# hellozhuo/svnet

Hardware: AMD Instinct MI355X
Metric: point-clouds/sec fwd+bwd, sv_dgcnn_cls B=32 N=1024 k=20 (higher is better)
Workload: dtype f32 (ternary bit-planes in the binarized layers); 1 GPU; sv_dgcnn_cls --binary fwd+loss+bwd, B=32 per GPU, N=1024, k=20; global_batch=32, parallelism=dp1, collective=none (1 rank), rccl_world=1, launch=hipGraph replay, binlinear=i8_mfma (>= 1024 rows) + xnor (head)

## Files before the change

include/svnet_hip.h:

```cpp
#ifndef SVNET_HIP_H
#define SVNET_HIP_H

#include <stddef.h>
#include <stdint.h>

#ifdef __cplusplus
extern "C" {
#endif

#define SVNET_OK 0
#define SVNET_E_ARG (-1)
#define SVNET_E_UNSUPPORTED (-2)
#define SVNET_E_WORKSPACE (-3)
#define SVNET_E_LAUNCH (-4)

#define SVNET_RED_SLICES 16
#define SVNET_SLICED_LEN(L) ((SVNET_RED_SLICES + 1) * (L) + 2)
int svnet_slices_sum_f32(float* buf, int64_t L, void* stream);
int svnet_slices_sum_f64(double* buf, int64_t L, void* stream);

#define SVNET_ABI_VERSION 425
int svnet_version(void);
const char* svnet_last_error(void);

typedef struct svnet_gate_fwd_job {
    const float* gin; const double* gin_f64; float* gin_out; float in_scale; const float* W0; const float* W2;
    int64_t B, Cin, H, Ov; float* h; float* gate;
    const float* rows; int64_t R;
} svnet_gate_fwd_job;
typedef struct svnet_gate_bwd_job {
    const float* dgate; const float* gate; const float* h; const float* gin; float in_scale; const float* W0; const float* W2;
    int64_t B, Cin, H, Ov; float out_scale; float* dgin; float* dW0; float* dW2;
} svnet_gate_bwd_job;

size_t svnet_knn_workspace_bytes(int64_t B, int64_t N, int64_t C);
int svnet_knn_f32(const float* x, int64_t B, int64_t N, int64_t C, int64_t sb, int64_t sn, int64_t sc,
                  int xx_mode, int k, int64_t* idx_out, void* workspace, size_t workspace_bytes, void* stream);
int svnet_knn_sv_f32(const float* s, int64_t Cs, const float* v, int64_t Cv3, int64_t B, int64_t N, int k, int64_t* idx_out,
                     void* workspace, size_t workspace_bytes, void* stream);

int svnet_knn_table_fusable(int64_t B, int64_t N, int64_t C);
int svnet_knn_from_table_f32(const void* workspace, size_t workspace_bytes, int64_t B, int64_t N, int64_t C, int k, int64_t* idx_out,
                             void* stream);
int svnet_edgeblock_apply_knn_f32(const int32_t* n_max, const int32_t* n_min, const float* mv, const float* mvn, const float* coef,
                                  const float* gate, int64_t P, int64_t N, int64_t Os, int64_t Ov, float slope, float* s_out, float* v_out,
                                  float* s_cat, int64_t s_ld, float* v_cat, int64_t v_ld, void* knn_workspace, size_t knn_workspace_bytes,
                                  void* stream);
int svnet_xyzblock_apply_knn_f32(const float* y_max, const float* y_min, const float* mv, const float* mvn, const float* coef,
                                 const float* gate, int64_t P, int64_t N, int64_t Os, int64_t Ov, float slope, float* s_out, float* v_out,
                                 float* s_cat, int64_t s_ld, float* v_cat, int64_t v_ld, void* knn_workspace, size_t knn_workspace_bytes,
                                 void* stream);

int svnet_edge_xyz_f32(const float* x, const int64_t* idx, int64_t B, int64_t N, int64_t k, int64_t m, int mode,
                       float* out, void* stream);

int svnet_edge_diffcat_fwd_f32(const float* table, const int64_t* idx, int idx_is_global, int64_t B, int64_t N,
                               int64_t k, int64_t G, int64_t F, float* out, void* stream);
int svnet_edge_diffcat_bwd_f32(const float* d_out, const int64_t* idx, int idx_is_global, int64_t B, int64_t N,
                               int64_t k, int64_t G, int64_t F, float* d_table, void* stream);

typedef struct svnet_gemm_desc {
    int64_t M, N, K;
    const float* A; int64_t a_rs, a_cs;
    const float* a_scale;
    const uint64_t* a_sign; const uint64_t* a_nz;
    const float* B; int64_t b_rs, b_cs;
    int b_exact;
    float* C; int64_t ldc, c_cs;
    float alpha;
    const float* col_scale;
    const float* bias;
    const uint64_t* mask;
    float* col_sum;
    int split_k;
// ... 391 lines not shown
```

svnet_amd/_ops.py:

```python
import ctypes

import torch

from . import _lib, config
from ._lib import BinHeadDesc, GemmDesc, call

BN_EPS = 1e-5
RED_SLICES = _lib.DEFINES["SVNET_RED_SLICES"]
BN_MOMENTUM = 0.1

TAP = None



def _p(t):
    return None if t is None else ctypes.c_void_p(t.data_ptr())


def _stream():
    return ctypes.c_void_p(torch.cuda.current_stream().cuda_stream)


def _hip(*tensors):
    for t in tensors:
# ... 1679 lines not shown
              and all(torch.is_tensor(b[0]) and torch.is_tensor(b[1]) and a[0] == b[0].data_ptr() and a[1] == b[1].data_ptr()
                      for a, b in zip(self.filled, levels)))
        if not ok:
            return torch.cat([x[0] for x in levels], dim=-1), torch.cat([x[1] for x in levels], dim=-1)
        flat = [t for vw in self.views for t in vw]
        return _CatFilled.apply(self.s, self.v, len(levels), *flat)


_SINK = None


class _CatFilled(torch.autograd.Function):

    @staticmethod
    def forward(ctx, s_cat, v_cat, n, *flat):
        ctx.ws = [flat[2 * i].shape[-1] for i in range(n)]
        ctx.wv = [flat[2 * i + 1].shape[-1] for i in range(n)]
        return s_cat.view(s_cat.shape), v_cat.view(v_cat.shape)

    @staticmethod
    def backward(ctx, gs, gv):
        out, so, vo = [], 0, 0
        for ws, wv in zip(ctx.ws, ctx.wv):
            out.append(gs[..., so:so + ws] if gs is not None else None)
            out.append(gv[..., vo:vo + wv] if gv is not None else None)
            so, vo = so + ws, vo + wv
        return (None, None, None) + tuple(out)


class EdgeBlock(torch.autograd.Function):

    @staticmethod
    def forward(ctx, s, v, idx, k, training, Wz, scz, W1, beta1, scale1, g1, b1, rm1, rv1, W2, sc2, g2, b2, rm2, rv2, Wg0, Wg2,
                nbt1=None, nbt2=None):
        _hip(s, v)
        from ._lib import EdgeBlockDesc
        s = _f32c(s)
        v = _f32c(v)
        B, N, Cs = s.shape
        Cv = v.shape[-1]
        Os, Ov = W1.shape[0], W2.shape[0]
        P, E = B * N, B * N * k
        dev = s.device
        f32 = dict(dtype=torch.float32, device=dev)
        W1c, W2c, Wzc, Wg0c, Wg2c = _f32c(W1), _f32c(W2), _f32c(Wz), _f32c(Wg0), _f32c(Wg2)
        sc1, sc2f, sczf = _f32c(scale1).reshape(-1), _f32c(sc2).reshape(-1), _f32c(scz).reshape(-1)

        import weakref
        refs = tuple(weakref.ref(p_) for p_ in (W1, beta1, W2, sc2, Wz, scz))

        def build():
            out = {"wv": torch.empty((2 * Ov + 6, Cv), **f32), "scv": torch.empty((2 * Ov + 6,), **f32),
                   "w_sign": torch.empty((Os, 5), dtype=torch.int64, device=dev), "w_nz": torch.empty((Os, 5), dtype=torch.int64, device=dev),
                   "beta_perm": torch.empty((5 * 64,), **f32), "wbt": torch.empty((320 * ((Os + 15) // 16 * 16),), dtype=torch.int16, device=dev),
                   "w_dense": torch.zeros((1,), dtype=torch.int32, device=dev)}

            def rebuild():
                ps = [r() for r in refs]
                if any(p_ is None for p_ in ps):
                    return
                W1p, beta1p, W2p, sc2p, Wzp, sczp = ps
                call("svnet_edgeblock_prepare_vec_f32", _p(_f32c(W2p.detach())), _p(_f32c(sc2p.detach()).reshape(-1)), _p(_f32c(Wzp.detach())),
                     _p(_f32c(sczp.detach()).reshape(-1)), Ov, Cv, _p(out["wv"]), _p(out["scv"]), _stream())
                call("svnet_edgeblock_prepare_f32", _p(_f32c(W1p.detach())), _p(_f32c(beta1p.detach())), Os, Cs, Cv, _p(out["w_sign"]), _p(out["w_nz"]),
                     _p(out["beta_perm"]), _stream())
                call("svnet_edgeblock_wbt_bf16", _p(out["w_sign"]), _p(out["w_nz"]), Os, Cs, Cv, _p(out["wbt"]), _p(out["w_dense"]), _stream())
            rebuild()
            return out, rebuild
        packed = PLANES.get("edge", (W1, beta1, W2, sc2, Wz, scz), build)
        wv, scv, w_sign, w_nz, beta_perm, wbt = (packed[n] for n in ("wv", "scv", "w_sign", "w_nz", "beta_perm", "wbt"))
        zz = torch.empty((P * 3, 6), **f32)
        ut = torch.empty((P * 3, 2 * Ov), **f32)
        main, side = torch.cuda.current_stream(dev), _side_stream(dev)
        side.wait_stream(main)
        idx = (idx if torch.is_tensor(idx) else idx.idx).contiguous()
        _hip(idx)
        with torch.cuda.stream(side):
            gemm(3 * P, 6, Cv, A=v, a_rs=Cv, a_cs=1, B=wv[2 * Ov:], b_rs=1, b_cs=Cv, b_exact=True, C=zz, ldc=6, col_scale=scv[2 * Ov:])
            gemm(3 * P, 2 * Ov, Cv, A=v, a_rs=Cv, a_cs=1, B=wv, b_rs=1, b_cs=Cv, b_exact=True, C=ut, ldc=2 * Ov, col_scale=scv)
        main.wait_stream(side)

        n_max = torch.empty((P, Os), dtype=torch.int32, device=dev)
        n_min = torch.empty((P, Os), dtype=torch.int32, device=dev)
        slot_max = torch.empty((P, Os), dtype=torch.uint8, device=dev)
        slot_min = torch.empty((P, Os), dtype=torch.uint8, device=dev)
        mv = torch.empty((P, 3, Ov), **f32)
        mvn = torch.empty((P, 3, Ov), **f32)
        if training:
            stat_n, stat_v, gate_sum = _zeros_pool(dev, ((RED_SLICES * 2 * Os,), torch.int64), ((RED_SLICES * 2 * Ov,), torch.float64),
                                                     ((B, 2 * Cs), torch.float64))
        else:
            stat_n = stat_v = None
            gate_sum = _zeros((B, 2 * Cs), torch.float64, dev)
        d = EdgeBlockDesc()
        d.B, d.N, d.k = B, N, k
        d.Cs, d.Cv, d.Os, d.Ov = Cs, Cv, Os, Ov
        d.s, d.v, d.idx, d.zz, d.ut = _p(s), _p(v), _p(idx), _p(zz), _p(ut)
        d.w_sign, d.w_nz, d.beta_perm = _p(w_sign), _p(w_nz), _p(beta_perm)
        d.w_dense = _p(packed["w_dense"]) if config.EDGE_DENSE_WEIGHTS else None
        d.n_max, d.n_min, d.slot_max, d.slot_min = _p(n_max), _p(n_min), _p(slot_max), _p(slot_min)
        d.mv, d.mvn, d.stat_n, d.stat_v, d.gate_sum = _p(mv), _p(mvn), _p(stat_n), _p(stat_v), _p(gate_sum)
        keep = (training and any(ctx.needs_input_grad)) or TAP is not None
        n16 = torch.empty((E, Os), dtype=torch.int16, device=dev) if keep else None
        planes = torch.empty((E, 15), dtype=torch.int64, device=dev) if keep else None
        d.n16, d.planes = _p(n16), _p(planes)
        call("svnet_edgeblock_fwd_f32", ctypes.byref(d), _stream())
        if TAP is not None:
# ... 263 lines not shown
```

svnet_amd/csrc/edgeblock_bwd.hip:

```cpp
#include <stdlib.h>

#include "bf16_split.h"
#include "common.h"
#include "gate_mlp.h"
#include "prelude.h"

namespace {

#define ATOMIC_ADD(p, v) do { if (MODE != 1) atomicAdd((p), (v)); else asm volatile("" :: "v"(v)); } while (0)

#ifdef SVNET_PHASE_CLOCK
#define PHASE_MARK(i) do { if (threadIdx.x == 0) { const long long t_ = clock64(); ph_acc[i] += (unsigned long long)(t_ - ph_t); ph_t = t_; } } while (0)
#define PHASE_INIT() __shared__ unsigned long long ph_acc[16]; long long ph_t = 0, ph_t0 = 0, ph_w0 = 0; \
    if (threadIdx.x == 0) { for (int i_ = 0; i_ < 16; ++i_) ph_acc[i_] = 0ull; ph_t = ph_t0 = clock64(); ph_w0 = wall_clock64(); }
#define PHASE_FLUSH() do { if (threadIdx.x == 0 && d.debug) { ph_acc[14] = (unsigned long long)(clock64() - ph_t0); \
        ph_acc[15] = (unsigned long long)(wall_clock64() - ph_w0); for (int i_ = 0; i_ < 16; ++i_) if (ph_acc[i_]) \
        atomicAdd(reinterpret_cast<unsigned long long*>(d.debug) + 8 + 16 * (blockIdx.x & 255) + i_, ph_acc[i_]); } } while (0)
#else
#define PHASE_MARK(i) do { } while (0)
#define PHASE_INIT() do { } while (0)
#define PHASE_FLUSH() do { } while (0)
#endif

typedef __attribute__((ext_vector_type(16))) float f32x16;

#ifndef SVNET_DN_PIECES
#define SVNET_DN_PIECES 3
#endif

constexpr float VEPS = 1e-6f;
constexpr int NW = 5;
constexpr int NCOL = NW * 64;
constexpr int TE = 32;
__host__ __device__ __forceinline__ int dx_stride(int Cs, int Cv) { return (2 * Cs + 6 * Cv) | 1; }

__host__ __device__ __forceinline__ int dn_stride(int Os) { return Os + 8; }

__device__ __forceinline__ int nth_set_bit10(uint32_t mask, int n) {
    int res = -1;
#pragma unroll
    for (int b = 9; b >= 0; --b) {
        const int below = __popc(mask & ((1u << b) - 1u));
        if (((mask >> b) & 1u) && below == n) res = b;
    }
    return res;
}
__global__ void edgeblock_wbt_kernel(const uint64_t* __restrict__ w_sign, const uint64_t* __restrict__ w_nz, int Os, int Cs, int Cv,
                                     uint16_t* __restrict__ wbt, uint32_t* __restrict__ w_dense) {
    if (w_dense && blockIdx.x == 0 && threadIdx.x < 64) {
        bool ok = true;
        for (int i = threadIdx.x; i < Os * NW; i += 64) {
            const int w = i % NW, nb = w < 2 ? Cs : 2 * Cv;
            const uint64_t used = nb >= 64 ? ~0ull : ((1ull << nb) - 1ull);
            ok = ok && ((w_nz[i] & used) == used);
        }
        const uint64_t bad = __ballot(!ok);
        if (threadIdx.x == 0) *w_dense = bad == 0ull ? 1u : 0u;
    }
    const int nks = (Os + 15) >> 4;
    const int total = (NCOL / 32) * nks * 512;
    for (int e = blockIdx.x * blockDim.x + threadIdx.x; e < total; e += gridDim.x * blockDim.x) {
        const int j = e & 7, ln = (e >> 3) & 63, rest = e >> 9;
        const int ct = rest / nks, ks = rest - ct * nks;
        const int col = ct * 32 + (ln & 31), o = ks * 16 + 8 * (ln >> 5) + j;
        const int w = col >> 6, b = col & 63;
        uint16_t val = 0;
        if (o < Os) {
            const uint64_t nz = w_nz[o * NW + w], sg = w_sign[o * NW + w];
            val = ((nz >> b) & 1ull) ? (((sg >> b) & 1ull) ? 0x3F80 : 0xBF80) : 0;
        }
        wbt[e] = val;
    }
}

__global__ __launch_bounds__(256) void edgeblock_bwd_prelude_kernel(
    const float* __restrict__ gs, const float* __restrict__ gv, const int32_t* __restrict__ n_max, const int32_t* __restrict__ n_min,
    const float* __restrict__ mv, const float* __restrict__ mvn, const float* __restrict__ coef, const float* __restrict__ scale1,
    const float* __restrict__ gate, int64_t P, int64_t N, int Os, int Ov, float slope, int64_t rows_per_block,
    float* __restrict__ gy, float* __restrict__ red, float* __restrict__ redv, float* __restrict__ dgate,
    const float* __restrict__ gs2, int64_t gs2_ld, const float* __restrict__ gv2, int64_t gv2_ld, float* __restrict__ gv_sum) {
    svnet_prelude_body<int32_t>(gs, gv, n_max, n_min, mv, mvn, coef, scale1, gate, P, N, Os, Ov, slope, rows_per_block, gy, red, redv, dgate, gs2,
                                gs2_ld, gv2, gv2_ld, gv_sum);
}

__global__ void edgeblock_bwd_coeffs_kernel(const float* __restrict__ red, const float* __restrict__ redv, const float* __restrict__ coef,
                                            const float* __restrict__ g1, const float* __restrict__ g2, int64_t E, int Os, int Ov,
                                            int training, const float* __restrict__ scale1, float* __restrict__ bcoef,
                                            float* __restrict__ dg1, float* __restrict__ db1, float* __restrict__ dg2,
                                            float* __restrict__ db2, svnet_gate_bwd_job job, int coef_blocks, int gate_chunks) {
    if ((int)blockIdx.x >= coef_blocks) {
        const int g = (int)blockIdx.x - coef_blocks;
        svnet_gate_bwd_block(job, g / gate_chunks, g % gate_chunks, gate_chunks);
        return;
    }
    const int c = blockIdx.x * blockDim.x + threadIdx.x;
    const float invE = 1.f / (float)E;
    if (c < Os) {
        const float iy = coef[3 * Os + c];
        float r0 = 0.f, r1 = 0.f;
#pragma unroll
        for (int sl = 0; sl < SVNET_RED_SLICES; ++sl) { r0 += red[sl * 2 * Os + c]; r1 += red[sl * 2 * Os + Os + c]; }
        const float m1 = training ? r0 * invE : 0.f, m2 = training ? r1 * invE : 0.f, cs = g1[c] * iy;
        bcoef[c] = m1;
        bcoef[Os + c] = m2;
        bcoef[2 * Os + c] = cs;
        dg1[c] = r1;
        db1[c] = r0;
        if (scale1) {
            float* chc = bcoef + ((3 * Os + 2 * Ov + 3) & ~3);
            const float sc = scale1[c], my = coef[2 * Os + c];
            chc[c] = cs;
            chc[Os + c] = cs * (m1 - my * iy * m2);
            chc[2 * Os + c] = cs * sc * iy * m2;
            chc[3 * Os + c] = sc;
            chc[4 * Os + c] = coef[c] >= 0.f ? 1.f : 0.f;
        }
    }
    if (c < Ov) {
        const float* Avp = coef + 4 * Os;
        const float mean = Avp[2 * Ov + c], is = Avp[3 * Ov + c];
// ... 174 lines not shown
    in.gp = in_range ? c.gp : 0u;
    if (in_range && c.gp != loaded_p) { load_point(d, c.gp, v2_lane, cm, pend); loaded_p = c.gp; }
    in.gj = in.valid ? c.b * N + (uint32_t)jloc : 0u;
    const uint32_t ld = (uint32_t)min(lane, (int)Cv - 1);
    const float* vj = d.v + in.gj * 3u * Cv;
    in.vj0 = ld_f32_sbase(vj, 4u * ld);
    in.vj1 = ld_f32_sbase(vj, 4u * (ld + Cv));
    in.vj2 = ld_f32_sbase(vj, 4u * (ld + 2u * Cv));
    const float* zj = d.zz + in.gj * 18u;
    in.zj[0] = zj[0];  in.zj[1] = zj[1];  in.zj[2] = zj[2];
    in.zj[3] = zj[6];  in.zj[4] = zj[7];  in.zj[5] = zj[8];
    in.zj[6] = zj[12]; in.zj[7] = zj[13]; in.zj[8] = zj[14];
}

#define SVNET_PHASEC_REQUESTS()                                                                             \
    do {                                                                                                    \
            const uint32_t Nu_ = (uint32_t)d.N, uCv_ = (uint32_t)Cv; \
            const int row0_ = 8 * wave, n3_ = 3 * Cv; \
            { \
                EdgeCursor c2; \
                cursor_init(d, tp, e0, row0_, c2); \
_Pragma("unroll") \
                for (int rr = 0; rr < 8; ++rr) { \
                    const int jl = __builtin_amdgcn_readlane(jv8, rr); \
                    const bool ok = c2.e < E && (uint32_t)jl < Nu_; \
                    const uint32_t gj = ok ? c2.b * Nu_ + (uint32_t)jl : 0u; \
                    const float* vr = d.v + gj * 3u * uCv_; \
                    pc_vst[rr][0] = ld_f32_sbase(vr, 4u * (uint32_t)min(lane, n3_ - 1)); \
                    if (NC2 > 44) pc_vst[rr][1] = ld_f32_sbase(vr, 4u * (uint32_t)min(lane + 64, n3_ - 1)); \
                    cursor_next(d, c2); \
                } \
            } \
            const int el_ = lane >> 3, ch_ = (lane >> 2) & 1, qq_ = min(lane & 3, 2); \
            const int rw_ = row0_ + el_; \
            const bool in_range_ = e0 + rw_ < E; \
            const uint32_t dq_ = small_div((uint32_t)(tp.t0 + rw_), tp.kmagic); \
            int pin_ = tp.pin0 + (int)dq_; \
            uint32_t b_ = tp.b0; \
            while (pin_ >= (int)Nu_) { pin_ -= (int)Nu_; ++b_; } \
            const int jloc_ = __builtin_amdgcn_ds_bpermute(4 * el_, jv8); \
            const bool valid_ = in_range_ && (uint32_t)jloc_ < Nu_; \
            const uint32_t gj_ = valid_ ? b_ * Nu_ + (uint32_t)jloc_ : 0u; \
            const uint32_t gpc_ = in_range_ ? tp.gp0 + dq_ : 0u; \
            const float* vip_ = d.v + (gpc_ * 3u + (uint32_t)qq_) * uCv_; \
_Pragma("unroll") \
            for (int i = 0; i < PC_NCH; ++i) pc_vi[i] = vip_[min(ch_ * PC_NCH + i, Cv - 1)]; \
            const float* zjp_ = d.zz + gj_ * 18u + (uint32_t)qq_ * 6u; \
            const float* zip_ = d.zz + gpc_ * 18u + (uint32_t)qq_ * 6u; \
            pc_zj[0] = zjp_[0]; pc_zj[1] = zjp_[1]; pc_zj[2] = zjp_[2]; \
_Pragma("unroll") \
            for (int i = 0; i < 6; ++i) pc_zi[i] = zip_[i]; \
    } while (0)

template <int MODE, int NKS, int NC2 = 0>
__global__ __launch_bounds__(256, 4) void edgeblock_bwd_kernel(svnet_edgeblock_bwd_desc d) {
    const uint32_t tile_lin = blockIdx.x;
    extern __shared__ __attribute__((aligned(16))) unsigned char smem[];
    const int Cs = d.Cs, Cv = d.Cv, Os = d.Os;
    const int DNB = dn_stride(Os);
    const int DXS = dx_stride(Cs, Cv);
    const int dx_floats = max(TE * DXS, (3 * TE * DNB + 1) / 2);
    float* dxl = reinterpret_cast<float*>(smem);
    uint16_t* dnb = reinterpret_cast<uint16_t*>(smem);
    uint64_t* pl = reinterpret_cast<uint64_t*>(dxl + ((dx_floats + 3) & ~3));

    PHASE_INIT();
    const int tid = threadIdx.x, lane = tid & 63;
    const int wave = __builtin_amdgcn_readfirstlane(tid >> 6);
    const int64_t E = d.B * d.N * d.k;
    uint32_t tile = tile_lin;
    const uint32_t nk = (uint32_t)d.N * (uint32_t)d.k;
    const uint32_t tpc = nk / TE;
    if ((d.B & 7) == 0 && tpc * TE == nk) {
        const uint32_t xcd = tile & 7u, slot = tile >> 3;
        const uint32_t sq = slot / tpc;
        tile = (sq * 8u + xcd) * tpc + (slot - sq * tpc);
    }
    const int64_t e0 = (int64_t)tile * TE;
    const int64_t ew = e0 + wave * (TE / 4);
    TilePos tp;
    {
        const uint32_t ku = (uint32_t)d.k, Nu = (uint32_t)d.N, e0u = tile * (uint32_t)TE;
        tp.gp0 = e0u / ku;
        tp.t0 = (int)(e0u - tp.gp0 * ku);
        tp.b0 = tp.gp0 / Nu;
        tp.pin0 = (int)(tp.gp0 - tp.b0 * Nu);
        tp.kmagic = (65536u + ku - 1u) / ku;
    }

    const bool v2_lane = lane < 2 * Cv, diff_lane = lane < Cv;
    const int cm = diff_lane ? lane : lane - Cv;
    const int jv8 = reinterpret_cast<const int*>(d.idx)[2 * min(ew + (lane & 7), E - 1)];

    uint32_t used_tiles = 0;
#pragma unroll
    for (int ct = 0; ct < NCOL / 32; ++ct) {
        const int width = (ct >> 1) < 2 ? Cs : 2 * Cv;
        if (width > 32 * (ct & 1)) used_tiles |= 1u << ct;
    }
    int cts[3];
#pragma unroll
    for (int q = 0; q < 3; ++q) cts[q] = __builtin_amdgcn_readfirstlane(nth_set_bit10(used_tiles, wave + 4 * q));

    const int nks = (Os + 15) >> 4;
    constexpr int NKB = NKS < 4 ? NKS : 4;
    bf16x8 bfr[NKB][3];
#define SVNET_LOAD_BFR(KS0)                                                                                    \
    do {                                                                                                       \
        const bf16x8* wbt_ = reinterpret_cast<const bf16x8*>(d.w1bt);            \
        _Pragma("unroll") for (int kb = 0; kb < NKB; ++kb)                                                     \
            _Pragma("unroll") for (int q = 0; q < 3; ++q) {                                                    \
                const int ct = cts[q], ks_ = (KS0) + kb;                                                       \
                if (ks_ < nks && ct >= 0) {                                                                    \
                    bfr[kb][q] = wbt_[(ct * nks + ks_) * 64 + lane];                                           \
                } else {                                                                                       \
                    _Pragma("unroll") for (int j = 0; j < 8; ++j) bfr[kb][q][j] = bf16_from_bits(0);           \
                }                                                                                              \
            }                                                                                                  \
    } while (0)
    constexpr bool HOIST_B = NKS <= 4;
    if (HOIST_B) SVNET_LOAD_BFR(0);
    float gc_pre0 = 0.f, gc_pre1 = 0.f;
    if constexpr (NC2 > 0) {
        const int sl_ = min(lane, Cs - 1);
        gc_pre0 = d.gconst[tp.b0 * 2u * (uint32_t)Cs + sl_];
        gc_pre1 = d.gconst[tp.b0 * 2u * (uint32_t)Cs + Cs + sl_];
    }

    {
        static_assert(TE * 3 * NW <= 512, "two plane words per thread");
        uint64_t plw[2];
#pragma unroll
        for (int u = 0; u < 2; ++u) {
            const int item = min(tid + 256 * u, TE * 3 * NW - 1);
            const int r = item / (3 * NW);
            plw[u] = d.planes[min(e0 + r, E - 1) * (3 * NW) + (item - r * (3 * NW))];
        }
        const int O4 = Os >> 2;
        const int o4_shift = __builtin_ctz((unsigned)O4);
        const int k = (int)d.k;
        const float* chc = d.bcoef + ((3 * Os + 2 * d.Ov + 3) & ~3);
        const int o4c = (tid & (O4 - 1)) << 2;
        const float4 cs = *reinterpret_cast<const float4*>(chc + o4c);
        const float4 al = *reinterpret_cast<const float4*>(chc + Os + o4c);
        const float4 be = *reinterpret_cast<const float4*>(chc + 2 * Os + o4c);
        const float4 sc = *reinterpret_cast<const float4*>(chc + 3 * Os + o4c);
        const float4 ps = *reinterpret_cast<const float4*>(chc + 4 * Os + o4c);
        constexpr int NI = NKS / 2;
        uint2 n4[NI]; float4 gy4[NI]; uint32_t smx[NI], smn[NI]; int tt[NI];
#pragma unroll
        for (int it = 0; it < NI; ++it) {
            const int item = it * 256 + tid;
            const int r = item >> o4_shift, o4 = (item & (O4 - 1)) << 2;
            const int64_t e = e0 + r;
            tt[it] = -1;
            if (item < TE * O4 && e < E) {
                const uint32_t n_ = (uint32_t)(tp.t0 + r), dq_ = small_div(n_, tp.kmagic);
                const int64_t gp = (int64_t)(tp.gp0 + dq_);
                tt[it] = (int)(n_ - dq_ * (uint32_t)k);
                n4[it] = *reinterpret_cast<const uint2*>(d.n16 + e * Os + o4);
                gy4[it] = *reinterpret_cast<const float4*>(d.gy + gp * Os + o4);
                smx[it] = *reinterpret_cast<const uint32_t*>(d.slot_max + gp * Os + o4);
                smn[it] = *reinterpret_cast<const uint32_t*>(d.slot_min + gp * Os + o4);
            }
        }
        __builtin_amdgcn_sched_barrier(0);
#pragma unroll
        for (int u = 0; u < 2; ++u) {
            const int item = tid + 256 * u;
            if (item < TE * 3 * NW) {
                const int r = item / (3 * NW), q = item - r * (3 * NW);
                const int plane = q / NW, w = q - plane * NW;
                pl[(plane * TE + r) * NW + w] = (e0 + r < E) ? plw[u] : 0ull;
            }
        }
        PHASE_MARK(11);
        __syncthreads();
        PHASE_MARK(12);
#pragma unroll
        for (int it = 0; it < NI; ++it) {
            const int item = it * 256 + tid;
            if (item >= TE * O4) break;
            const int r = item >> o4_shift, o4 = (item & (O4 - 1)) << 2;
            const int64_t e = e0 + r;
            const int t = tt[it];
            float4 dn = make_float4(0.f, 0.f, 0.f, 0.f);
            if (Os == 8 && o4 == 0) {
#pragma unroll
                for (int p = 0; p < 3; ++p) *reinterpret_cast<uint4*>(dnb + (p * TE + r) * DNB + 8) = make_uint4(0u, 0u, 0u, 0u);
            }
            if (t >= 0) {
                const uint32_t sx = smx[it], sn = smn[it];
                const float g0 = ((int)((ps.x != 0.f ? sx : sn) & 0xFFu) == t) ? gy4[it].x : 0.f;
                const float g1 = ((int)(((ps.y != 0.f ? sx : sn) >> 8) & 0xFFu) == t) ? gy4[it].y : 0.f;
                const float g2 = ((int)(((ps.z != 0.f ? sx : sn) >> 16) & 0xFFu) == t) ? gy4[it].z : 0.f;
                const float g3 = ((int)((ps.w != 0.f ? sx : sn) >> 24) == t) ? gy4[it].w : 0.f;
                const float n0 = (float)(short)(n4[it].x & 0xFFFFu), n1 = (float)((int)n4[it].x >> 16);
                const float n2 = (float)(short)(n4[it].y & 0xFFFFu), n3 = (float)((int)n4[it].y >> 16);
                float4 dy;
                dy.x = cs.x * g0 - (al.x + be.x * n0);
                dy.y = cs.y * g1 - (al.y + be.y * n1);
                dy.z = cs.z * g2 - (al.z + be.z * n2);
                dy.w = cs.w * g3 - (al.w + be.w * n3);
                if (d.dn_out) *reinterpret_cast<float4*>(d.dn_out + e * Os + o4) = dy;
                dn = make_float4(dy.x * sc.x, dy.y * sc.y, dy.z * sc.z, dy.w * sc.w);
            }
            uint32_t h0, m0, l0, h1, m1, l1;
            split3_pair(dn.x, dn.y, h0, m0, l0);
            split3_pair(dn.z, dn.w, h1, m1, l1);
            uint16_t* o_ = dnb + r * DNB + o4;
            *reinterpret_cast<uint2*>(o_) = make_uint2(h0, h1);
            *reinterpret_cast<uint2*>(o_ + TE * DNB) = make_uint2(m0, m1);
#if SVNET_DN_PIECES >= 3
            *reinterpret_cast<uint2*>(o_ + 2 * TE * DNB) = make_uint2(l0, l1);
#endif
        }
    }
    __syncthreads();
    PHASE_MARK(0);
    if (MODE == 2) { PHASE_FLUSH(); return; }

    {
        const int64_t word_row = e0 >> 6;
        const int half = (int)((e0 >> 5) & 1);
        if (Cs <= 32 && 2 * Cv <= 32) {
            for (int pi = wave; pi < NW; pi += 4) {
                const int ent = 2 * pi + (lane >> 5);
                const int plane = ent / NW, w = ent - plane * NW;
                const uint32_t mine = (uint32_t)pl[(plane * TE + (lane & 31)) * NW + w];
                const uint32_t colword = svnet_bit_transpose32(mine, lane);
                uint32_t* dst = plane == 0 ? d.x_sign32 : d.x_nz32;
                dst[((word_row * NCOL) + w * 64 + (lane & 31)) * 2 + half] = colword;
            }
        } else
        for (int item = wave; item < 2 * NW; item += 4) {
            const int plane = item / NW, w = item - plane * NW;
            const uint64_t roww = pl[(plane * TE + (lane & 31)) * NW + w];
            const uint32_t mine = lane < 32 ? (uint32_t)roww : (uint32_t)(roww >> 32);
            const uint32_t colword = svnet_bit_transpose32(mine, lane);
            uint32_t* dst = plane == 0 ? d.x_sign32 : d.x_nz32;
            dst[((word_row * NCOL) + w * 64 + lane) * 2 + half] = colword;
        }
    }

    PHASE_MARK(1);
    constexpr int PC_NCH = NC2 > 0 ? NC2 / 4 : 1;
    float pc_vst[8][2], pc_vi[PC_NCH], pc_zj[3], pc_zi[6];
    {
        const int r = lane & 31, h = lane >> 5;
        f32x16 acc[3];
#pragma unroll
        for (int q = 0; q < 3; ++q)
#pragma unroll
            for (int i = 0; i < 16; ++i) acc[q][i] = 0.f;
#pragma unroll
        for (int ks0 = 0; ks0 < NKS; ks0 += NKB) {
            if (!HOIST_B) SVNET_LOAD_BFR(ks0);
#pragma unroll
            for (int kb = 0; kb < NKB; ++kb) {
                const int ks = ks0 + kb;
                if (ks < nks) {
                    const uint16_t* a_ = dnb + r * DNB + ks * 16 + 8 * h;
                    const bf16x8 fh = *reinterpret_cast<const bf16x8*>(a_), fm = *reinterpret_cast<const bf16x8*>(a_ + TE * DNB);
#if SVNET_DN_PIECES >= 3
                    const bf16x8 fl = *reinterpret_cast<const bf16x8*>(a_ + 2 * TE * DNB);
#endif
#pragma unroll
                    for (int q = 0; q < 3; ++q) {
                        if (cts[q] >= 0) {
                            acc[q] = __builtin_amdgcn_mfma_f32_32x32x16_bf16(fh, bfr[kb][q], acc[q], 0, 0, 0);
                            acc[q] = __builtin_amdgcn_mfma_f32_32x32x16_bf16(fm, bfr[kb][q], acc[q], 0, 0, 0);
#if SVNET_DN_PIECES >= 3
                            acc[q] = __builtin_amdgcn_mfma_f32_32x32x16_bf16(fl, bfr[kb][q], acc[q], 0, 0, 0);
#endif
                        }
                    }
                }
            }
        }
        PHASE_MARK(5);
        if constexpr (NC2 > 0 && NKS >= 4) SVNET_PHASEC_REQUESTS();
        __syncthreads();
        PHASE_MARK(6);
#pragma unroll
        for (int q = 0; q < 3; ++q) {
            const int ct = cts[q];
            if (ct >= 0) {
                const int col = ct * 32 + r;
                const int wd = ct >> 1, wi = (ct & 1) * 32 + r;
                const bool in_use = wi < (wd < 2 ? Cs : 2 * Cv);
                const int ccol = (wd < 2 ? wd * Cs : 2 * Cs + (wd - 2) * 2 * Cv) + wi;
                const uint32_t roww = reinterpret_cast<const uint32_t*>(pl)[((2 * TE + r) * NW + wd) * 2 + (ct & 1)];
                const int cmask = (int)(svnet_bit_transpose32(roww, lane) >> (4 * h));
                float csum = 0.f;
#pragma unroll
                for (int i = 0; i < 16; ++i) {
                    const int rb = (i & 3) + 8 * (i >> 2), row = rb + 4 * h;
                    const uint32_t keep = (uint32_t)__builtin_amdgcn_sbfe(cmask, rb, 1);
                    const float v = __uint_as_float(__float_as_uint(acc[q][i]) & keep);
                    if (in_use) dxl[row * DXS + ccol] = v;
                    csum += v;
                }
                const float other = lane_half_swap(csum);
                if (h == 0 && in_use) { const float t = csum + other; if (t != 0.f) ATOMIC_ADD(&d.dbeta_perm[(tile_lin & (SVNET_DBETA_SLICES - 1)) * NCOL + col], t); }
            }
        }
    }
    __syncthreads();
    PHASE_MARK(2);
    if (MODE == 3) { PHASE_FLUSH(); return; }

    if constexpr (NC2 > 0) {
        constexpr int NCH = NC2 / 4;
        constexpr int RW = 8;
        const int64_t R = msg_stride(Cs, Cv, d.Ov);
        const uint32_t Nu = (uint32_t)d.N, uCv = (uint32_t)Cv;
        const int row0 = RW * wave;
        const int n3 = 3 * Cv;
        float* zs = reinterpret_cast<float*>(pl);
        EdgeCursor cur;
        cursor_init(d, tp, e0, row0, cur);

        if constexpr (NKS < 4) SVNET_PHASEC_REQUESTS();
        float (&vst)[RW][2] = pc_vst;
        const int el = lane >> 3, ch = (lane >> 2) & 1, q = lane & 3, qq = min(q, 2);
        const int r = row0 + el;
        const int64_t e = e0 + r;
        const bool in_range = e < E;
        const int jloc = __builtin_amdgcn_ds_bpermute(4 * el, jv8);
        const bool valid = in_range && (uint32_t)jloc < Nu;
        if (in_range && !valid && d.debug && (lane & 7) == 0) {
            if (atomicAdd(reinterpret_cast<unsigned long long*>(d.debug), 1ull) == 0ull) { d.debug[1] = e; d.debug[2] = jloc; d.debug[3] = d.N; }
        }
        const int c0 = ch * NCH;
        float (&vi)[NCH] = pc_vi;
        const float zj0 = pc_zj[0], zj1 = pc_zj[1], zj2 = pc_zj[2];
        const float zi0 = pc_zi[0], zi1 = pc_zi[1], zi2 = pc_zi[2], zi3 = pc_zi[3], zi4 = pc_zi[4], zi5 = pc_zi[5];

        PHASE_MARK(10);
        {
            const bool s_lane = lane < Cs;
            const int sl = min(lane, Cs - 1);
            uint32_t cur_p = 0xFFFFFFFFu, cur_b = 0xFFFFFFFFu;
            float g0c = 0.f, g1c = 0.f, cs_sum = 0.f;
            EdgeCursor c2 = cur;
            for (int rr = 0; rr < RW; ++rr) {
                if (c2.e >= E) break;
                if (c2.gp != cur_p) {
                    if (cur_p != 0xFFFFFFFFu && s_lane) ATOMIC_ADD(&d.ds_acc[cur_p * (uint32_t)Cs + (uint32_t)lane], cs_sum);
                    cur_p = c2.gp;
                    cs_sum = 0.f;
                    if (c2.b != cur_b) {
                        cur_b = c2.b;
                        if (cur_b == tp.b0) { g0c = gc_pre0; g1c = gc_pre1; }
// ... 155 lines not shown
                for (int q9 = 0; q9 < 9; ++q9) zc[q9] = pend.zi[(q9 / 3) * 6 + 3 + q9 % 3] - pend.zi[(q9 / 3) * 6 + q9 % 3];
            }
            cursor_next(d, cur);
            load_edge(d, cur, __builtin_amdgcn_readlane(jv8, min(rr + 2, TE / 4 - 1)), rr + 2 < TE / 4 ? E : 0, lane, v2_lane, cm,
                      q[(u + 2) & 3], pend, loaded_p);
            const float* row = dxl + r * DXS;
            if (in.in_range) {
                const float d0 = row[sl] + g0c;
                if (s_lane) {
                    st_f32_sbase(srow0 + (uint32_t)rr * (uint32_t)R, 4u * (uint32_t)lane, d0);
                    cs_sum += (row[Cs + sl] + g1c) - d0;
                }
            }
            const bool live = v2_lane && in.valid;
            const float g0 = live ? row[2 * Cs + lane] : 0.f, g1 = live ? row[2 * Cs + 2 * Cv + lane] : 0.f,
                        g2 = live ? row[2 * Cs + 4 * Cv + lane] : 0.f;
            const float z0 = in.zj[0] + zc[0], z1 = in.zj[1] + zc[1], z2 = in.zj[2] + zc[2], z3 = in.zj[3] + zc[3], z4 = in.zj[4] + zc[4],
                        z5 = in.zj[5] + zc[5], z6 = in.zj[6] + zc[6], z7 = in.zj[7] + zc[7], z8 = in.zj[8] + zc[8];
            const float ve0 = diff_lane ? (in.vj0 - vi0) : (v2_lane ? vi0 : 0.f);
            const float ve1 = diff_lane ? (in.vj1 - vi1) : (v2_lane ? vi1 : 0.f);
            const float ve2 = diff_lane ? (in.vj2 - vi2) : (v2_lane ? vi2 : 0.f);
            const float dve0 = g0 * z0 + g1 * z1 + g2 * z2;
            const float dve1 = g0 * z3 + g1 * z4 + g2 * z5;
            const float dve2 = g0 * z6 + g1 * z7 + g2 * z8;
            const float pz[8] = {g0 * ve0, g1 * ve0, g2 * ve0, g0 * ve1, g1 * ve1, g2 * ve1, g0 * ve2, g1 * ve2};
            const float dzp = wave_sum8_packed(pz, lane);
            const float dz8 = wave_sum_last(g2 * ve2);
            czq += dzp;
            czq8 += dz8;
            if (diff_lane) { cvd0 -= dve0; cvd1 -= dve1; cvd2 -= dve2; }
            else if (v2_lane) { cvd0 += dve0; cvd1 += dve1; cvd2 += dve2; }
            if (in.valid) {
                float* m = mrow0 + (uint32_t)rr * (uint32_t)R;
                if (diff_lane) { st_f32_sbase(m, bo_d0, dve0); st_f32_sbase(m, bo_d1, dve1); st_f32_sbase(m, bo_d2, dve2); }
                if (zq_writer) st_f32_sbase(m, bo_zq, dzp);
                if (lane == 63) st_f32_sbase(m, bo_z8, dz8);
            }
        }
        }
        if (cur_p != 0xFFFFFFFFu) SVNET_FLUSH_POINT(cur_p);
#undef SVNET_FLUSH_POINT
#undef SVNET_LOAD_BFR
    }
    PHASE_MARK(4);
    PHASE_FLUSH();
}

}

extern "C" int svnet_edgeblock_wbt_bf16(const uint64_t* w_sign, const uint64_t* w_nz, int64_t Os, int64_t Cs, int64_t Cv, uint16_t* wbt,
                                        uint32_t* w_dense, void* stream) {
    SVNET_REQUIRE(w_sign && w_nz && wbt && Os > 0 && Os % 8 == 0, SVNET_E_ARG, "svnet_edgeblock_wbt_bf16: bad arguments (Os must be a multiple of 8)");
    SVNET_REQUIRE(!w_dense || (Cs > 0 && Cs <= 64 && Cv > 0 && 2 * Cv <= 64), SVNET_E_ARG, "svnet_edgeblock_wbt_bf16: w_dense needs the layer's Cs <= 64, 2 Cv <= 64");
    hipLaunchKernelGGL(edgeblock_wbt_kernel, dim3((unsigned)svnet_cdiv(NCOL * ((Os + 15) / 16 * 16), 256)), dim3(256), 0, (hipStream_t)stream, w_sign, w_nz,
                       (int)Os, (int)Cs, (int)Cv, wbt, w_dense);
    SVNET_CHECK_LAUNCH("edgeblock_wbt_kernel");
    return SVNET_OK;
}

extern "C" int svnet_edgeblock_bwd_prelude_f32(const float* gs, const float* gv, const int32_t* n_max, const int32_t* n_min,
                                               const float* mv, const float* mvn, const float* coef, const float* scale1,
                                               const float* gate, int64_t P, int64_t N, int64_t Os, int64_t Ov, float slope,
                                               float* gy, float* red, float* redv, float* dgate, const float* gs2, int64_t gs2_ld,
                                               const float* gv2, int64_t gv2_ld, float* gv_sum, void* stream) {
    SVNET_REQUIRE((gs || gs2) && (gv || gv2) && n_max && n_min && mv && mvn && coef && scale1 && gate && gy && red && redv && dgate, SVNET_E_ARG,
                  "svnet_edgeblock_bwd_prelude_f32: null pointer");
    SVNET_REQUIRE((!gs2 || gs2_ld >= Os) && (!gv2 || (gv2_ld >= Ov && gv_sum)), SVNET_E_ARG,
                  "svnet_edgeblock_bwd_prelude_f32: second gradient source needs row strides >= the slice and gv_sum");
    SVNET_REQUIRE(P > 0 && N > 0 && Os > 0 && Ov > 0, SVNET_E_ARG, "svnet_edgeblock_bwd_prelude_f32: bad sizes");
    SVNET_REQUIRE(Os <= 128 && Ov <= 64, SVNET_E_UNSUPPORTED, "svnet_edgeblock_bwd_prelude_f32: Os <= 128, Ov <= 64");
    const int64_t rpb = svnet_prelude_rows(N);
    hipLaunchKernelGGL(edgeblock_bwd_prelude_kernel, dim3((unsigned)svnet_cdiv(P, rpb)), dim3(256), 0, (hipStream_t)stream, gs, gv, n_max,
                       n_min, mv, mvn, coef, scale1, gate, P, N, (int)Os, (int)Ov, slope, rpb, gy, red, redv, dgate, gs2, gs2_ld, gv2, gv2_ld,
                       gv_sum);
    SVNET_CHECK_LAUNCH("edgeblock_bwd_prelude_kernel");
    return SVNET_OK;
}

extern "C" int svnet_edgeblock_bwd_coeffs_f32(const float* red, const float* redv, const float* coef, const float* gamma1,
                                              const float* gamma2, int64_t E, int64_t Os, int64_t Ov, int training, const float* scale1,
                                              float* bcoef, float* dgamma1, float* dbeta1, float* dgamma2, float* dbeta2,
                                              const svnet_gate_bwd_job* gate_job, void* stream) {
    SVNET_REQUIRE(red && redv && coef && gamma1 && gamma2 && bcoef && dgamma1 && dbeta1 && dgamma2 && dbeta2 && E > 0, SVNET_E_ARG,
                  "svnet_edgeblock_bwd_coeffs_f32: bad arguments");
    const int64_t n = Os > Ov ? Os : Ov;
    SVNET_REQUIRE(!gate_job || svnet_gate_bwd_job_ok(gate_job), SVNET_E_ARG, "svnet_edgeblock_bwd_coeffs_f32: bad gate job");
    const int coef_blocks = (int)svnet_cdiv(n, 256);
    const svnet_gate_bwd_job job = gate_job ? *gate_job : svnet_gate_bwd_job{};
    const int chunks = gate_job ? svnet_gate_bwd_chunks(job.Cin, job.H, job.Ov) : 1;
    hipLaunchKernelGGL(edgeblock_bwd_coeffs_kernel, dim3((unsigned)(coef_blocks + (gate_job ? gate_job->B * chunks : 0))), dim3(256), 0,
                       (hipStream_t)stream, red, redv, coef, gamma1, gamma2, E, (int)Os, (int)Ov, training, scale1, bcoef, dgamma1, dbeta1,
                       dgamma2, dbeta2, job, coef_blocks, chunks);
    SVNET_CHECK_LAUNCH("edgeblock_bwd_coeffs_kernel");
    return SVNET_OK;
}

extern "C" int svnet_edgeblock_bwd_tier(int64_t Cs, int64_t Cv, int64_t Os) {
    if (!(Cs > 0 && Cs <= 64 && Cv > 0 && 2 * Cv <= 64 && Os >= 8 && Os <= 128 && (Os & (Os - 1)) == 0)) return -1;
    const int nks = Os <= 32 ? 2 : Os <= 64 ? 4 : 8;
    const bool c8 = Cv >= 3 && Cv <= 24 && 3 * Cv <= 2 * Cs && 3 * Cv <= 128;
    return 100 * nks + (!c8 ? 0 : Cv <= 10 ? 20 : Cv <= 12 ? 24 : Cv <= 21 ? 44 : 48);
}

extern "C" int svnet_edgeblock_bwd_f32(const svnet_edgeblock_bwd_desc* desc, void* stream) {
    SVNET_REQUIRE(desc, SVNET_E_ARG, "svnet_edgeblock_bwd_f32: null descriptor");
    const svnet_edgeblock_bwd_desc& d = *desc;
    SVNET_REQUIRE(d.v && d.idx && d.zz && d.ut && d.n16 && d.planes && d.w1bt && d.scale1 && d.slot_max && d.slot_min && d.coef &&
// ... 64 lines not shown
```

Before: 7769 point-clouds/sec.

## Hoist edgeblock bwd global loads, pipeline B fragments, tune occupancy per config

The edgeblock backward kernel now issues its plane, n16, coefficient, gy and slot loads at kernel entry using scalar-base plus offset addressing with clamped rows. This is meant to overlap their latency with the tile-position setup. B-fragment loads become branchless by appending a zero fragment to the packed weight buffer, and are software-pipelined one step ahead inside the MFMA loop. Launch-bounds occupancy and the number of column tiles per wave (NQ) are specialised for the NC2=20/24 configurations, and LDS stores use readfirstlane row offsets. The trade-off is higher register pressure and a larger wbt buffer.

```diff
diff --git a/include/svnet_hip.h b/include/svnet_hip.h
--- a/include/svnet_hip.h
+++ b/include/svnet_hip.h
@@ -19,7 +19,7 @@
 int svnet_slices_sum_f32(float* buf, int64_t L, void* stream);
 int svnet_slices_sum_f64(double* buf, int64_t L, void* stream);
 
-#define SVNET_ABI_VERSION 425
+#define SVNET_ABI_VERSION 426
 int svnet_version(void);
 const char* svnet_last_error(void);
 
diff --git a/svnet_amd/_ops.py b/svnet_amd/_ops.py
--- a/svnet_amd/_ops.py
+++ b/svnet_amd/_ops.py
@@ -1755,7 +1755,7 @@
         def build():
             out = {"wv": torch.empty((2 * Ov + 6, Cv), **f32), "scv": torch.empty((2 * Ov + 6,), **f32),
                    "w_sign": torch.empty((Os, 5), dtype=torch.int64, device=dev), "w_nz": torch.empty((Os, 5), dtype=torch.int64, device=dev),
-                   "beta_perm": torch.empty((5 * 64,), **f32), "wbt": torch.empty((320 * ((Os + 15) // 16 * 16),), dtype=torch.int16, device=dev),
+                   "beta_perm": torch.empty((5 * 64,), **f32), "wbt": torch.empty((320 * ((Os + 15) // 16 * 16) + 512,), dtype=torch.int16, device=dev),
                    "w_dense": torch.zeros((1,), dtype=torch.int32, device=dev)}
 
             def rebuild():
diff --git a/svnet_amd/csrc/edgeblock_bwd.hip b/svnet_amd/csrc/edgeblock_bwd.hip
--- a/svnet_amd/csrc/edgeblock_bwd.hip
+++ b/svnet_amd/csrc/edgeblock_bwd.hip
@@ -24,6 +24,11 @@
 
 typedef __attribute__((ext_vector_type(16))) float f32x16;
 
+template <typename T>
+__device__ __forceinline__ T ld_sbase(const void* base, uint32_t byte_off) {
+    return *reinterpret_cast<const T*>(reinterpret_cast<const char*>(base) + keep_here(byte_off));
+}
+
 #ifndef SVNET_DN_PIECES
 #define SVNET_DN_PIECES 3
 #endif
@@ -58,14 +63,14 @@
         if (threadIdx.x == 0) *w_dense = bad == 0ull ? 1u : 0u;
     }
     const int nks = (Os + 15) >> 4;
-    const int total = (NCOL / 32) * nks * 512;
+    const int total = (NCOL / 32 * nks + 1) * 512;
     for (int e = blockIdx.x * blockDim.x + threadIdx.x; e < total; e += gridDim.x * blockDim.x) {
         const int j = e & 7, ln = (e >> 3) & 63, rest = e >> 9;
         const int ct = rest / nks, ks = rest - ct * nks;
         const int col = ct * 32 + (ln & 31), o = ks * 16 + 8 * (ln >> 5) + j;
         const int w = col >> 6, b = col & 63;
         uint16_t val = 0;
-        if (o < Os) {
+        if (o < Os && ct < NCOL / 32) {
             const uint64_t nz = w_nz[o * NW + w], sg = w_sign[o * NW + w];
             val = ((nz >> b) & 1ull) ? (((sg >> b) & 1ull) ? 0x3F80 : 0xBF80) : 0;
         }
@@ -346,8 +351,10 @@
             for (int i = 0; i < 6; ++i) pc_zi[i] = zip_[i]; \
     } while (0)
 
+constexpr int tile_waves(int NKS, int NC2) { return (NC2 != 20 && NC2 != 24) ? 4 : NKS == 2 ? 6 : NKS == 4 ? 5 : 4; }
+
 template <int MODE, int NKS, int NC2 = 0>
-__global__ __launch_bounds__(256, 4) void edgeblock_bwd_kernel(svnet_edgeblock_bwd_desc d) {
+__global__ __launch_bounds__(256, tile_waves(NKS, NC2)) void edgeblock_bwd_kernel(svnet_edgeblock_bwd_desc d) {
     const uint32_t tile_lin = blockIdx.x;
     extern __shared__ __attribute__((aligned(16))) unsigned char smem[];
     const int Cs = d.Cs, Cv = d.Cv, Os = d.Os;
@@ -372,6 +379,35 @@
     }
     const int64_t e0 = (int64_t)tile * TE;
     const int64_t ew = e0 + wave * (TE / 4);
+    const int rows_in = (int)min((int64_t)TE, E - e0);
+
+    const int jv8 = ld_sbase<int>(d.idx + e0, 8u * (uint32_t)min(8 * wave + (lane & 7), rows_in - 1));
+    static_assert(TE * 3 * NW <= 512, "two plane words per thread");
+    uint64_t plw[2];
+#pragma unroll
+    for (int u = 0; u < 2; ++u) {
+        const int item = min(tid + 256 * u, TE * 3 * NW - 1);
+        const int r = item / (3 * NW);
+        plw[u] = ld_sbase<uint64_t>(d.planes + e0 * (3 * NW), 8u * (uint32_t)(min(r, rows_in - 1) * (3 * NW) + (item - r * (3 * NW))));
+    }
+    const int O4 = Os >> 2;
+    const int o4_shift = __builtin_ctz((unsigned)O4);
+    constexpr int NI = NKS / 2;
+    uint2 n4[NI]; float4 gy4[NI]; uint32_t smx[NI], smn[NI]; int tt[NI];
+#pragma unroll
+    for (int it = 0; it < NI; ++it) {
+        const int item = it * 256 + tid;
+        const int rc = min(item >> o4_shift, rows_in - 1), o4 = (item & (O4 - 1)) << 2;
+        n4[it] = ld_sbase<uint2>(d.n16 + e0 * Os, 2u * (uint32_t)(rc * Os + o4));
+    }
+    const float* chc = d.bcoef + ((3 * Os + 2 * d.Ov + 3) & ~3);
+    const uint32_t o4c = 16u * (uint32_t)(tid & (O4 - 1));
+    const float4 cs = ld_sbase<float4>(chc, o4c);
+    const float4 al = ld_sbase<float4>(chc + Os, o4c);
+    const float4 be = ld_sbase<float4>(chc + 2 * Os, o4c);
+    const float4 sc = ld_sbase<float4>(chc + 3 * Os, o4c);
+    const float4 ps = ld_sbase<float4>(chc + 4 * Os, o4c);
+    __builtin_amdgcn_sched_barrier(0);
     TilePos tp;
     {
         const uint32_t ku = (uint32_t)d.k, Nu = (uint32_t)d.N, e0u = tile * (uint32_t)TE;
@@ -381,10 +417,20 @@
         tp.pin0 = (int)(tp.gp0 - tp.b0 * Nu);
         tp.kmagic = (65536u + ku - 1u) / ku;
     }
+#pragma unroll
+    for (int it = 0; it < NI; ++it) {
+        const int item = it * 256 + tid;
+        const int r = item >> o4_shift, rc = min(r, rows_in - 1), o4 = (item & (O4 - 1)) << 2;
+        const uint32_t n_ = (uint32_t)(tp.t0 + rc), dq_ = small_div(n_, tp.kmagic);
+        tt[it] = (item < TE * O4 && r < rows_in) ? (int)(n_ - dq_ * (uint32_t)d.k) : -1;
+        const uint32_t po = dq_ * (uint32_t)Os + (uint32_t)o4;
+        gy4[it] = ld_sbase<float4>(d.gy + (int64_t)tp.gp0 * Os, 4u * po);
+        smx[it] = ld_sbase<uint32_t>(d.slot_max + (int64_t)tp.gp0 * Os, po);
+        smn[it] = ld_sbase<uint32_t>(d.slot_min + (int64_t)tp.gp0 * Os, po);
+    }
 
     const bool v2_lane = lane < 2 * Cv, diff_lane = lane < Cv;
     const int cm = diff_lane ? lane : lane - Cv;
-    const int jv8 = reinterpret_cast<const int*>(d.idx)[2 * min(ew + (lane & 7), E - 1)];
 
     uint32_t used_tiles = 0;
 #pragma unroll
@@ -392,28 +438,27 @@
         const int width = (ct >> 1) < 2 ? Cs : 2 * Cv;
         if (width > 32 * (ct & 1)) used_tiles |= 1u << ct;
     }
-    int cts[3];
-#pragma unroll
-    for (int q = 0; q < 3; ++q) cts[q] = __builtin_amdgcn_readfirstlane(nth_set_bit10(used_tiles, wave + 4 * q));
+    constexpr int NQ = (NC2 == 20 || NC2 == 24) ? 2 : 3;
+    int cts[NQ];
+#pragma unroll
+    for (int q = 0; q < NQ; ++q) cts[q] = __builtin_amdgcn_readfirstlane(nth_set_bit10(used_tiles, wave + 4 * q));
 
     const int nks = (Os + 15) >> 4;
     constexpr int NKB = NKS < 4 ? NKS : 4;
-    bf16x8 bfr[NKB][3];
-#define SVNET_LOAD_BFR(KS0)                                                                                    \
+    bf16x8 bfr[NKB][NQ];
+    const int zfrag = (NCOL / 32) * nks;
+#define SVNET_LOAD_BFR(KB, KS)                                                                                 \
     do {                                                                                                       \
-        const bf16x8* wbt_ = reinterpret_cast<const bf16x8*>(d.w1bt);            \
-        _Pragma("unroll") for (int kb = 0; kb < NKB; ++kb)                                                     \
-            _Pragma("unroll") for (int q = 0; q < 3; ++q) {                                                    \
-                const int ct = cts[q], ks_ = (KS0) + kb;                                                       \
-                if (ks_ < nks && ct >= 0) {                                                                    \
-                    bfr[kb][q] = wbt_[(ct * nks + ks_) * 64 + lane];                                           \
-                } else {                                                                                       \
-                    _Pragma("unroll") for (int j = 0; j < 8; ++j) bfr[kb][q][j] = bf16_from_bits(0);           \
-                }                                                                                              \
-            }                                                                                                  \
+        _Pragma("unroll") for (int q = 0; q < NQ; ++q) {                                                       \
+            const int fi_ = (cts[q] >= 0 && (NKS > 2 || (KS) < nks)) ? cts[q] * nks + (KS) : zfrag;            \
+            bfr[KB][q] = ld_sbase<bf16x8>(d.w1bt + (uint32_t)fi_ * 512u, 16u * (uint32_t)lane);                \
+        }                                                                                                      \
     } while (0)
     constexpr bool HOIST_B = NKS <= 4;
-    if (HOIST_B) SVNET_LOAD_BFR(0);
+    if (HOIST_B) {
+#pragma unroll
+        for (int kb = 0; kb < NKB; ++kb) SVNET_LOAD_BFR(kb, kb);
+    }
     float gc_pre0 = 0.f, gc_pre1 = 0.f;
     if constexpr (NC2 > 0) {
         const int sl_ = min(lane, Cs - 1);
@@ -422,42 +467,6 @@
     }
 
     {
-        static_assert(TE * 3 * NW <= 512, "two plane words per thread");
-        uint64_t plw[2];
-#pragma unroll
-        for (int u = 0; u < 2; ++u) {
-            const int item = min(tid + 256 * u, TE * 3 * NW - 1);
-            const int r = item / (3 * NW);
-            plw[u] = d.planes[min(e0 + r, E - 1) * (3 * NW) + (item - r * (3 * NW))];
-        }
-        const int O4 = Os >> 2;
-        const int o4_shift = __builtin_ctz((unsigned)O4);
-        const int k = (int)d.k;
-        const float* chc = d.bcoef + ((3 * Os + 2 * d.Ov + 3) & ~3);
-        const int o4c = (tid & (O4 - 1)) << 2;
-        const float4 cs = *reinterpret_cast<const float4*>(chc + o4c);
-        const float4 al = *reinterpret_cast<const float4*>(chc + Os + o4c);
-        const float4 be = *reinterpret_cast<const float4*>(chc + 2 * Os + o4c);
-        const float4 sc = *reinterpret_cast<const float4*>(chc + 3 * Os + o4c);
-        const float4 ps = *reinterpret_cast<const float4*>(chc + 4 * Os + o4c);
-        constexpr int NI = NKS / 2;
-        uint2 n4[NI]; float4 gy4[NI]; uint32_t smx[NI], smn[NI]; int tt[NI];
-#pragma unroll
-        for (int it = 0; it < NI; ++it) {
-            const int item = it * 256 + tid;
-            const int r = item >> o4_shift, o4 = (item & (O4 - 1)) << 2;
-            const int64_t e = e0 + r;
-            tt[it] = -1;
-            if (item < TE * O4 && e < E) {
-                const uint32_t n_ = (uint32_t)(tp.t0 + r), dq_ = small_div(n_, tp.kmagic);
-                const int64_t gp = (int64_t)(tp.gp0 + dq_);
-                tt[it] = (int)(n_ - dq_ * (uint32_t)k);
-                n4[it] = *reinterpret_cast<const uint2*>(d.n16 + e * Os + o4);
-                gy4[it] = *reinterpret_cast<const float4*>(d.gy + gp * Os + o4);
-                smx[it] = *reinterpret_cast<const uint32_t*>(d.slot_max + gp * Os + o4);
-                smn[it] = *reinterpret_cast<const uint32_t*>(d.slot_min + gp * Os + o4);
-            }
-        }
         __builtin_amdgcn_sched_barrier(0);
 #pragma unroll
         for (int u = 0; u < 2; ++u) {
@@ -465,7 +474,7 @@
             if (item < TE * 3 * NW) {
                 const int r = item / (3 * NW), q = item - r * (3 * NW);
                 const int plane = q / NW, w = q - plane * NW;
-                pl[(plane * TE + r) * NW + w] = (e0 + r < E) ? plw[u] : 0ull;
+                pl[(plane * TE + r) * NW + w] = r < rows_in ? plw[u] : 0ull;
             }
         }
         PHASE_MARK(11);
@@ -476,7 +485,6 @@
             const int item = it * 256 + tid;
             if (item >= TE * O4) break;
             const int r = item >> o4_shift, o4 = (item & (O4 - 1)) << 2;
-            const int64_t e = e0 + r;
             const int t = tt[it];
             float4 dn = make_float4(0.f, 0.f, 0.f, 0.f);
             if (Os == 8 && o4 == 0) {
@@ -496,7 +504,7 @@
                 dy.y = cs.y * g1 - (al.y + be.y * n1);
                 dy.z = cs.z * g2 - (al.z + be.z * n2);
                 dy.w = cs.w * g3 - (al.w + be.w * n3);
-                if (d.dn_out) *reinterpret_cast<float4*>(d.dn_out + e * Os + o4) = dy;
+                if (d.dn_out) *reinterpret_cast<float4*>(reinterpret_cast<char*>(d.dn_out + e0 * Os) + keep_here(16u * (uint32_t)item)) = dy;
                 dn = make_float4(dy.x * sc.x, dy.y * sc.y, dy.z * sc.z, dy.w * sc.w);
             }
             uint32_t h0, m0, l0, h1, m1, l1;
@@ -514,6 +522,10 @@
     PHASE_MARK(0);
     if (MODE == 2) { PHASE_FLUSH(); return; }
 
+    if (!HOIST_B) {
+#pragma unroll
+        for (int kb = 0; kb < NKB; ++kb) SVNET_LOAD_BFR(kb, kb);
+    }
     {
         const int64_t word_row = e0 >> 6;
         const int half = (int)((e0 >> 5) & 1);
@@ -542,25 +554,24 @@
     float pc_vst[8][2], pc_vi[PC_NCH], pc_zj[3], pc_zi[6];
     {
         const int r = lane & 31, h = lane >> 5;
-        f32x16 acc[3];
-#pragma unroll
-        for (int q = 0; q < 3; ++q)
+        f32x16 acc[NQ];
+#pragma unroll
+        for (int q = 0; q < NQ; ++q)
 #pragma unroll
             for (int i = 0; i < 16; ++i) acc[q][i] = 0.f;
 #pragma unroll
         for (int ks0 = 0; ks0 < NKS; ks0 += NKB) {
-            if (!HOIST_B) SVNET_LOAD_BFR(ks0);
 #pragma unroll
             for (int kb = 0; kb < NKB; ++kb) {
                 const int ks = ks0 + kb;
-                if (ks < nks) {
+                if (NKS > 2 || ks < nks) {
                     const uint16_t* a_ = dnb + r * DNB + ks * 16 + 8 * h;
                     const bf16x8 fh = *reinterpret_cast<const bf16x8*>(a_), fm = *reinterpret_cast<const bf16x8*>(a_ + TE * DNB);
 #if SVNET_DN_PIECES >= 3
                     const bf16x8 fl = *reinterpret_cast<const bf16x8*>(a_ + 2 * TE * DNB);
 #endif
 #pragma unroll
-                    for (int q = 0; q < 3; ++q) {
+                    for (int q = 0; q < NQ; ++q) {
                         if (cts[q] >= 0) {
                             acc[q] = __builtin_amdgcn_mfma_f32_32x32x16_bf16(fh, bfr[kb][q], acc[q], 0, 0, 0);
                             acc[q] = __builtin_amdgcn_mfma_f32_32x32x16_bf16(fm, bfr[kb][q], acc[q], 0, 0, 0);
@@ -570,14 +581,19 @@
                         }
                     }
                 }
+                if (ks + NKB < NKS) SVNET_LOAD_BFR(kb, ks + NKB);
             }
         }
         PHASE_MARK(5);
         if constexpr (NC2 > 0 && NKS >= 4) SVNET_PHASEC_REQUESTS();
         __syncthreads();
         PHASE_MARK(6);
-#pragma unroll
-        for (int q = 0; q < 3; ++q) {
+        int roff[16];
+#pragma unroll
+        for (int i = 0; i < 16; ++i) roff[i] = __builtin_amdgcn_readfirstlane(((i & 3) + 8 * (i >> 2)) * DXS);
+        const int hoff = 4 * h * DXS;
+#pragma unroll
+        for (int q = 0; q < NQ; ++q) {
             const int ct = cts[q];
             if (ct >= 0) {
                 const int col = ct * 32 + r;
@@ -587,13 +603,18 @@
                 const uint32_t roww = reinterpret_cast<const uint32_t*>(pl)[((2 * TE + r) * NW + wd) * 2 + (ct & 1)];
                 const int cmask = (int)(svnet_bit_transpose32(roww, lane) >> (4 * h));
                 float csum = 0.f;
+                float mv[16];
 #pragma unroll
                 for (int i = 0; i < 16; ++i) {
-                    const int rb = (i & 3) + 8 * (i >> 2), row = rb + 4 * h;
+                    const int rb = (i & 3) + 8 * (i >> 2);
                     const uint32_t keep = (uint32_t)__builtin_amdgcn_sbfe(cmask, rb, 1);
-                    const float v = __uint_as_float(__float_as_uint(acc[q][i]) & keep);
-                    if (in_use) dxl[row * DXS + ccol] = v;
-                    csum += v;
+                    mv[i] = __uint_as_float(__float_as_uint(acc[q][i]) & keep);
+                    csum += mv[i];
+                }
+                if (in_use) {
+                    float* const dcol = dxl + hoff + ccol;
+#pragma unroll
+                    for (int i = 0; i < 16; ++i) dcol[roff[i]] = mv[i];
                 }
                 const float other = lane_half_swap(csum);
                 if (h == 0 && in_use) { const float t = csum + other; if (t != 0.f) ATOMIC_ADD(&d.dbeta_perm[(tile_lin & (SVNET_DBETA_SLICES - 1)) * NCOL + col], t); }
@@ -855,7 +876,7 @@
                                         uint32_t* w_dense, void* stream) {
     SVNET_REQUIRE(w_sign && w_nz && wbt && Os > 0 && Os % 8 == 0, SVNET_E_ARG, "svnet_edgeblock_wbt_bf16: bad arguments (Os must be a multiple of 8)");
     SVNET_REQUIRE(!w_dense || (Cs > 0 && Cs <= 64 && Cv > 0 && 2 * Cv <= 64), SVNET_E_ARG, "svnet_edgeblock_wbt_bf16: w_dense needs the layer's Cs <= 64, 2 Cv <= 64");
-    hipLaunchKernelGGL(edgeblock_wbt_kernel, dim3((unsigned)svnet_cdiv(NCOL * ((Os + 15) / 16 * 16), 256)), dim3(256), 0, (hipStream_t)stream, w_sign, w_nz,
+    hipLaunchKernelGGL(edgeblock_wbt_kernel, dim3((unsigned)svnet_cdiv(NCOL * ((Os + 15) / 16 * 16) + 512, 256)), dim3(256), 0, (hipStream_t)stream, w_sign, w_nz,
                        (int)Os, (int)Cs, (int)Cv, wbt, w_dense);
     SVNET_CHECK_LAUNCH("edgeblock_wbt_kernel");
     return SVNET_OK;
```

After: 7968 point-clouds/sec, median of 6. +2.6%, better.
